# G1OJS/PyFT8

Hardware: AMD Instinct MI355X
Metric: FT8 15-s frames decoded/sec (higher is better)
Workload: dtype f32

## Files before the change

### pyft8_amd/csrc/kernels/common.hpp

```cpp
#ifndef FT8RX_COMMON_HPP
#define FT8RX_COMMON_HPP

struct Tables {
    const float* win;
    const cpx* W1920;
    const cpx* WR3840;
    const cpx* W3200;
    const cpx* W96000;
    const cpx* W300;
    const cpx* W320;
    const cpx* WR192k;
    const cpx* W32;
    const double* taper;
    const float* K32;
    const cpx* CS100;
    const cpx* TW100;
    const cpx* G1000;
};

__device__ __constant__ int d_COSTAS[7] = {3, 1, 4, 0, 6, 5, 2};
__device__ __constant__ uint8_t d_PAYSYM[58] = {7,8,9,10,11,12,13,14,15,16,17,18,19,20,21,22,23,24,25,26,27,28,29,30,31,32,33,34,35,
    43,44,45,46,47,48,49,50,51,52,53,54,55,56,57,58,59,60,61,62,63,64,65,66,67,68,69,70,71};
struct WorkList { int32_t* items; int32_t* count; };

constexpr __host__ __device__ int cand_shift(int max_cands) { return max_cands <= 256 ? 8 : max_cands <= 512 ? 9 : max_cands <= 1024 ? 10 : 11; }
constexpr __host__ __device__ int cand_shift(const ft8rx_config& c) { return cand_shift(c.max_cands); }
FT8_DEV bool cand_live(int c, int B, int sh, const int32_t* ncand) { return c < (B << sh) && (c & ((1 << sh) - 1)) < ncand[c >> sh]; }

FT8_DEV bool xcd_frame_map(int L, int per, int B, int& frame, int& idx) {
    const int x = L & 7, j = L >> 3;
    frame = 8 * (j / per) + x; idx = j % per;
    return frame < B;
}
#define XCD_GRID(B, per) ((((B) + 7) / 8) * 8 * (per))
enum { WL_BP0 = 0, WL_FINE = 1, WL_BP1 = 2, WL_BP1B = 3, WL_BP1C = 4, WL_OSD = 5, WL_OSDNAN = 6, WL_N = 7 };

#define W6 ((double)(-0.16666667163372040f))

#ifndef FT8RX_ILP_UNIT
__device__ __constant__ int8_t d_AP_CQ[29]   = {0,0,0,0,0, 0,0,0,0,0, 0,0,0,0,0, 0,0,0,0,0, 0,0,0,0,0, 0,1,0,0};
__device__ __constant__ int8_t d_AP_END[3][19] = {{0,1, 1,1,1,1,1, 0,0,1,1,1, 0,1,0,1,0, 0,1},
                                                  {0,1, 1,1,1,1,1, 0,1,0,0,1, 0,1,0,0,0, 0,1},
                                                  {0,1, 1,1,1,1,1, 0,1,0,0,1, 0,0,1,0,0, 0,1}};
__device__ uint8_t  d_CHK_N[83];
__device__ int16_t  d_CHK_V[83][7];
__device__ uint8_t  d_EDGE_V[522];
__device__ uint8_t  d_EDGE_C[522];
__device__ uint16_t d_VAR_E[174][3];
__device__ uint64_t d_G0[91][3];
__device__ uint64_t d_CHK_MASK[128][3];

struct Att {
    uint64_t lo, hi;
    int16_t n_its;
    uint8_t ok;
    uint8_t method;
    uint8_t nc0;
    uint8_t has_out;
    uint8_t pad[2];
};

FT8_DEV void work_push(const WorkList& w, int cand) { if (w.items) w.items[atomicAdd(w.count, 1)] = cand; }
FT8_DEV void work_push_block(const WorkList& w, bool want, int cand) {
    __shared__ int s_wave[4], s_base;
    const int lane = threadIdx.x & 63, wv = threadIdx.x >> 6;
    const uint64_t m = __ballot(want);
    if (lane == 0) s_wave[wv] = __popcll(m);
    __syncthreads();
    if (threadIdx.x == 0) {
        const int tot = s_wave[0] + s_wave[1] + s_wave[2] + s_wave[3];
        s_base = tot ? atomicAdd(w.count, tot) : 0;
    }
    __syncthreads();
    if (want) {
        int off = s_base + __popcll(m & ((1ull << lane) - 1));
        for (int i = 0; i < wv; i++) off += s_wave[i];
        w.items[off] = cand;
    }
}
FT8_DEV float grid_at(const float* __restrict__ g, int row, int col) {
    row %= 750; if (row < 0) row += 750;
    const bool in = row >= 1 && row <= 375;
    const uint32_t raw = __float_as_uint(g[(in ? row : 1) * FT8RX_GRID_COLS + col]);
    const uint32_t m = in ? 0xFFFFFFFFu : 0u;
    return __uint_as_float((raw & m) | (0x3F800000u & ~m));
}

FT8_DEV void log_event(ft8rx_event* ev, int32_t* evcount, int frame, int cand, int ipass, int slot, int seq,
                       uint64_t lo, uint64_t hi, int valid) {
    if (!ev) return;
    int idx = atomicAdd(&evcount[frame], 1);
    if (idx < FT8RX_EVENT_CAP) {
        ft8rx_event e; e.msg_lo = lo; e.msg_hi = hi; e.cand = (uint16_t)cand; e.ipass = (uint8_t)ipass;
        e.slot = (uint8_t)slot; e.seq = (uint16_t)seq; e.valid = (uint16_t)valid;
        ev[(size_t)frame * FT8RX_EVENT_CAP + idx] = e;
    }
}

__global__ __launch_bounds__(1024) void k_ev_scan(const int32_t* __restrict__ evcount, int B, int32_t* __restrict__ offs) {
    __shared__ int s_wave[16];
    __shared__ int s_carry;
    const int tid = threadIdx.x, lane = tid & 63, wv = tid >> 6;
    if (tid == 0) s_carry = 0;
    __syncthreads();
    for (int base = 0; base < B; base += 1024) {
        const int f = base + tid;
        int c = f < B ? evcount[f] : 0;
        c = c > FT8RX_EVENT_CAP ? FT8RX_EVENT_CAP : (c < 0 ? 0 : c);
        int incl = c;
#pragma unroll
        for (int d = 1; d < 64; d <<= 1) { const int t = __shfl_up(incl, d); if (lane >= d) incl += t; }
        if (lane == 63) s_wave[wv] = incl;
        __syncthreads();
        int before = s_carry;
        for (int i = 0; i < wv; i++) before += s_wave[i];
        if (f < B) offs[f] = before + incl - c;
        __syncthreads();
        if (tid == 1023) s_carry = before + incl;
        __syncthreads();
    }
    if (tid == 0) offs[B] = s_carry;
}
__global__ __launch_bounds__(64) void k_ev_compact(const ft8rx_event* __restrict__ ev, const int32_t* __restrict__ evcount,
                                                   const int32_t* __restrict__ offs, ft8rx_event* __restrict__ out) {
    const int f = blockIdx.x;
    int c = evcount[f]; c = c > FT8RX_EVENT_CAP ? FT8RX_EVENT_CAP : c;
    const uint32_t* src = reinterpret_cast<const uint32_t*>(ev + (size_t)f * FT8RX_EVENT_CAP);
    uint32_t* dst = reinterpret_cast<uint32_t*>(out + offs[f]);
    for (int i = threadIdx.x; i < c * 6; i += 64) dst[i] = src[i];
}

static_assert(sizeof(ft8rx_record) == 48 && sizeof(ft8rx_event) == 24 && sizeof(ft8rx_packed_frame) == 16 &&
              sizeof(ft8rx_packed_header) == 32, "packed result layout");
__global__ __launch_bounds__(256) void k_pack_count(const ft8rx_record* __restrict__ rec, const int32_t* __restrict__ ncand,
                                                    const ft8rx_event* __restrict__ ev, const int32_t* __restrict__ evcount,
                                                    uint64_t* __restrict__ need , int32_t* __restrict__ nrec , int sh) {
    __shared__ uint32_t s_has[FT8RX_MAX_CANDS / 32];
    __shared__ int s_cnt[FT8RX_MAX_CANDS / 64], s_nan;
    const int f = blockIdx.x, tid = threadIdx.x, lane = tid & 63, S = 1 << sh, nw = S >> 6;
    for (int i = tid; i < S / 32; i += 256) s_has[i] = 0;
    if (tid == 0) s_nan = 0;
    __syncthreads();
    int c = evcount[f]; c = c > FT8RX_EVENT_CAP ? FT8RX_EVENT_CAP : (c < 0 ? 0 : c);
    for (int i = tid; i < c; i += 256) {
        const unsigned cand = ev[(size_t)f * FT8RX_EVENT_CAP + i].cand;
        if (cand < (unsigned)S) atomicOr(&s_has[cand >> 5], 1u << (cand & 31));
    }
    int n = ncand[f]; n = n > S ? S : (n < 0 ? 0 : n);
    for (int i = tid; i < n; i += 256) {
        const ft8rx_record& r = rec[((size_t)f << sh) + i];
        if (r.grid_sd != r.grid_sd || r.fine_sd != r.fine_sd) s_nan = 1;
    }
    __syncthreads();
#pragma unroll 1
    for (int q = 0; q < S / 256; q++) {
        const int i = tid + 256 * q;
        const bool decoded = i < n && rec[((size_t)f << sh) + (i < n ? i : 0)].status == FT8RX_ST_DECODED;
        const bool want = i < n && (decoded || ((s_has[i >> 5] >> (i & 31)) & 1u) || s_nan);
        const uint64_t m = __ballot(want);
        if (lane == 0) { need[(size_t)f * nw + (i >> 6)] = m; s_cnt[i >> 6] = __popcll(m); }
    }
    __syncthreads();
    if (tid == 0) { int t = 0; for (int w = 0; w < nw; w++) t += s_cnt[w]; nrec[f] = t; }
}
__global__ __launch_bounds__(1024) void k_pack_scan(const int32_t* __restrict__ nrec, const int32_t* __restrict__ ncand,
                                                    const int32_t* __restrict__ evcount, int B, int max_cands, unsigned long long cap_bytes,
                                                    unsigned char* __restrict__ buf, ft8rx_packed_header* __restrict__ hdr_host) {
    __shared__ int s_wr[16], s_we[16];
    __shared__ int s_cr, s_ce;
    const int tid = threadIdx.x, lane = tid & 63, wv = tid >> 6;
    ft8rx_packed_frame* table = reinterpret_cast<ft8rx_packed_frame*>(buf + sizeof(ft8rx_packed_header));
    const bool table_fits = sizeof(ft8rx_packed_header) + (size_t)B * sizeof(ft8rx_packed_frame) <= cap_bytes;
    if (tid == 0) { s_cr = 0; s_ce = 0; }
    __syncthreads();
    for (int base = 0; base < B; base += 1024) {
        const int f = base + tid;
        const int r = f < B ? nrec[f] : 0;
        const int eraw = f < B ? evcount[f] : 0;
        const int e = eraw > FT8RX_EVENT_CAP ? FT8RX_EVENT_CAP : (eraw < 0 ? 0 : eraw);
        int ir = r, ie = e;
#pragma unroll
        for (int d = 1; d < 64; d <<= 1) { const int tr = __shfl_up(ir, d), te = __shfl_up(ie, d); if (lane >= d) { ir += tr; ie += te; } }
        if (lane == 63) { s_wr[wv] = ir; s_we[wv] = ie; }
        __syncthreads();
        int br = s_cr, be = s_ce;
        for (int i = 0; i < wv; i++) { br += s_wr[i]; be += s_we[i]; }
        if (f < B && table_fits) {
            ft8rx_packed_frame t;
            t.rec_off = br + ir - r; t.ev_off = be + ie - e;
            int n = ncand[f]; n = n > max_cands ? max_cands : (n < 0 ? 0 : n);
            t.n_cand = (uint16_t)n; t.n_rec = (uint16_t)r; t.n_ev = eraw < 0 ? 0 : eraw;
            table[f] = t;
        }
        __syncthreads();
        if (tid == 1023) { s_cr = br + ir; s_ce = be + ie; }
        __syncthreads();
    }
    if (tid == 0) {
        ft8rx_packed_header hd;
        hd.magic = FT8RX_PACKED_MAGIC; hd.n_frames = B; hd.n_records = s_cr; hd.n_events = s_ce; hd.max_cands = max_cands;
        hd.bytes = sizeof(ft8rx_packed_header) + (unsigned long long)B * sizeof(ft8rx_packed_frame) +
                   (unsigned long long)s_cr * sizeof(ft8rx_record) + (unsigned long long)s_ce * sizeof(ft8rx_event);
        hd.overflow = hd.bytes > cap_bytes;
        if (cap_bytes >= sizeof(hd)) *reinterpret_cast<ft8rx_packed_header*>(buf) = hd;
        *hdr_host = hd;
    }
}
__global__ __launch_bounds__(256) void k_pack_write(const ft8rx_record* __restrict__ rec, const ft8rx_event* __restrict__ ev,
                                                    const uint64_t* __restrict__ need, int B, unsigned char* __restrict__ buf, int sh) {
    const ft8rx_packed_header hd = *reinterpret_cast<const ft8rx_packed_header*>(buf);
    if (hd.overflow) return;
    __shared__ int s_pre[FT8RX_MAX_CANDS / 64];
    const int f = blockIdx.x, tid = threadIdx.x, lane = tid & 63, S = 1 << sh, nw = S >> 6;
    const ft8rx_packed_frame t = reinterpret_cast<const ft8rx_packed_frame*>(buf + sizeof(ft8rx_packed_header))[f];
    unsigned char* recs = buf + sizeof(ft8rx_packed_header) + (size_t)B * sizeof(ft8rx_packed_frame);
    unsigned char* evs = recs + (size_t)hd.n_records * sizeof(ft8rx_record);
    if (tid == 0) { int a = 0; for (int w = 0; w < nw; w++) { s_pre[w] = a; a += __popcll(need[(size_t)f * nw + w]); } }
    __syncthreads();
#pragma unroll 1
    for (int q = 0; q < S / 256; q++) {
        const int i = tid + 256 * q;
        const uint64_t mine = need[(size_t)f * nw + (i >> 6)];
        if ((mine >> lane) & 1ull) {
            const int p = s_pre[i >> 6] + __popcll(mine & ((1ull << lane) - 1));
            const uint4* src = reinterpret_cast<const uint4*>(rec + ((size_t)f << sh) + i);
            uint4* dst = reinterpret_cast<uint4*>(recs + ((size_t)t.rec_off + p) * sizeof(ft8rx_record));
            uint4 a = src[0], b = src[1], c = src[2];
            c.w = (uint32_t)i;
            dst[0] = a; dst[1] = b; dst[2] = c;
        }
    }
    const int ne = t.n_ev > FT8RX_EVENT_CAP ? FT8RX_EVENT_CAP : t.n_ev;
    const uint2* es = reinterpret_cast<const uint2*>(ev + (size_t)f * FT8RX_EVENT_CAP);
    uint2* ed = reinterpret_cast<uint2*>(evs + (size_t)t.ev_off * sizeof(ft8rx_event));
    for (int i = tid; i < ne * 3; i += 256) ed[i] = es[i];
}
#endif

#endif
```

### pyft8_amd/csrc/kernels/osd.hpp

```cpp
#ifndef FT8RX_OSD_HPP
#define FT8RX_OSD_HPP

#ifdef OSD_TIMING
__device__ unsigned long long g_osd_t[32768][10];
struct OsdClock { unsigned long long prev = __builtin_readcyclecounter(); };
#define OT(i) do { const unsigned long long ot_now = __builtin_readcyclecounter(); if (lane == 0) g_osd_t[blockIdx.x & 32767][i] += ot_now - ot.prev; ot.prev = __builtin_readcyclecounter(); } while (0)
#define OT_FLUSH do { if (lane == 0) g_osd_t[blockIdx.x & 32767][9] += 1ull; } while (0)
#else
struct OsdClock {};
#define OT(i) do { } while (0)
#define OT_FLUSH do { } while (0)
#endif
template <int M> FT8_DEV uint32_t osd_px(uint32_t v, int lane) {
    if (M == 1) return (uint32_t)__builtin_amdgcn_update_dpp(0, (int)v, 0xB1, 0xf, 0xf, false);
    if (M == 2) return (uint32_t)__builtin_amdgcn_update_dpp(0, (int)v, 0x4E, 0xf, 0xf, false);
    if (M == 3) return (uint32_t)__builtin_amdgcn_update_dpp(0, (int)v, 0x1B, 0xf, 0xf, false);
    if (M == 7) return (uint32_t)__builtin_amdgcn_update_dpp(0, (int)v, 0x141, 0xf, 0xf, false);
    if (M == 15) return (uint32_t)__builtin_amdgcn_update_dpp(0, (int)v, 0x140, 0xf, 0xf, false);
    if (M == 8) return (uint32_t)__builtin_amdgcn_update_dpp(0, (int)v, 0x128, 0xf, 0xf, false);
    if (M == 4 || M == 16 || M == 31) return (uint32_t)__builtin_amdgcn_ds_swizzle((int)v, 0x1f | (M << 10));
    return __shfl(v, lane ^ M);
}
#define OSD_LOWMASK(top) ((top) == 1 ? 0x5555555555555555ull : (top) == 2 ? 0x3333333333333333ull : (top) == 4 ? 0x0F0F0F0F0F0F0F0Full : \
                          (top) == 8 ? 0x00FF00FF00FF00FFull : (top) == 16 ? 0x0000FFFF0000FFFFull : 0x00000000FFFFFFFFull)
#define OSD_DPP_STAGE(CTRL)                                                                                                          \
    asm volatile("v_min_u32_dpp %[mn], %[hk], %[hk] " CTRL " row_mask:0xf bank_mask:0xf\n\t"                                         \
                 "v_max_u32_dpp %[mx], %[hk], %[hk] " CTRL " row_mask:0xf bank_mask:0xf\n\t"                                         \
                 "v_cndmask_b32 %[mn], %[mx], %[mn], %[low]\n\t"                                                                    \
                 "v_cmp_eq_u32 vcc, %[mn], %[hk]\n\t"                                                                                \
                 "s_nop 1\n\t"                                                                                                       \
                 "v_cndmask_b32_dpp %[ix], %[ix], %[ix], vcc " CTRL " row_mask:0xf bank_mask:0xf\n\t"                                \
                 : [mn] "=&v"(mn), [mx] "=&v"(mx), [ix] "+v"(ix[q]) : [hk] "v"(hk[q]), [low] "s"(low) : "vcc");
template <int M, int NQ> FT8_DEV void osd_stage(uint32_t* hk, uint32_t* ix, int lane) {
    constexpr int top = M >= 32 ? 32 : M >= 16 ? 16 : M >= 8 ? 8 : M >= 4 ? 4 : M >= 2 ? 2 : 1;
    const uint64_t low = OSD_LOWMASK(top);
#pragma unroll
    for (int q = 0; q < NQ; q++) {
        uint32_t mn, mx;
        if constexpr (M == 1) { OSD_DPP_STAGE("quad_perm:[1,0,3,2]") }
        else if constexpr (M == 2) { OSD_DPP_STAGE("quad_perm:[2,3,0,1]") }
        else if constexpr (M == 3) { OSD_DPP_STAGE("quad_perm:[3,2,1,0]") }
        else if constexpr (M == 7) { OSD_DPP_STAGE("row_half_mirror") }
        else if constexpr (M == 15) { OSD_DPP_STAGE("row_mirror") }
        else if constexpr (M == 8) { OSD_DPP_STAGE("row_ror:8") }
        else {
            const uint32_t pk = osd_px<M>(hk[q], lane), pi = osd_px<M>(ix[q], lane);
            mn = pk < hk[q] ? pk : hk[q]; mx = pk < hk[q] ? hk[q] : pk;
            asm("v_cndmask_b32 %0, %1, %0, %2" : "+v"(mn) : "v"(mx), "s"(low));
            ix[q] = (mn == hk[q]) ? ix[q] : pi;
        }
        hk[q] = mn;
    }
}
#undef OSD_DPP_STAGE
template <int NQ> FT8_DEV void osd_stages_421(uint32_t* hk, uint32_t* ix, int lane) {
    osd_stage<4, NQ>(hk, ix, lane); osd_stage<2, NQ>(hk, ix, lane); osd_stage<1, NQ>(hk, ix, lane);
}
template <bool REV> FT8_DEV void osd_stage_regs(uint32_t& ka, uint32_t& ia, uint32_t& kb, uint32_t& ib, int lane) {
    const uint32_t pkb = REV ? __shfl(kb, 63 - lane) : kb, pib = REV ? __shfl(ib, 63 - lane) : ib;
    const uint32_t pka = REV ? __shfl(ka, 63 - lane) : ka, pia = REV ? __shfl(ia, 63 - lane) : ia;
    const uint32_t na = pkb < ka ? pkb : ka, nb = pka > kb ? pka : kb;
    ia = (na == ka) ? ia : pib; ib = (nb == kb) ? ib : pia;
    ka = na; kb = nb;
}
#define FT8_HD __host__ __device__ inline
FT8_HD bool osd_nl(const float* x, int a, int b) {
    const float xa = x[a], xb = x[b];
    if (xa == xa && xb == xb) return fabsf(xa) > fabsf(xb);
    return xa == xa;
}
FT8_HD void osd_ss_linear_insert(const float* x, int* a, int last) {
    const int val = a[last]; int next = last - 1;
    while (osd_nl(x, val, a[next])) { a[last] = a[next]; last = next; next--; }
    a[last] = val;
}
FT8_HD void osd_ss_insertion(const float* x, int* a, int first, int last) {
    for (int i = first + 1; i < last; i++) {
        if (osd_nl(x, a[i], a[first])) { const int val = a[i]; for (int j = i; j > first; j--) a[j] = a[j - 1]; a[first] = val; }
        else osd_ss_linear_insert(x, a, i);
    }
}
FT8_HD void osd_ss_adjust_heap(const float* x, int* a, int first, int hole, int len, int value) {
    const int top = hole; int child = hole;
    while (child < (len - 1) / 2) {
        child = 2 * (child + 1);
        if (osd_nl(x, a[first + child], a[first + child - 1])) child--;
        a[first + hole] = a[first + child]; hole = child;
    }
    if ((len & 1) == 0 && child == (len - 2) / 2) { child = 2 * (child + 1); a[first + hole] = a[first + child - 1]; hole = child - 1; }
    int parent = (hole - 1) / 2;
    while (hole > top && osd_nl(x, a[first + parent], value)) { a[first + hole] = a[first + parent]; hole = parent; parent = (hole - 1) / 2; }
    a[first + hole] = value;
}
FT8_HD void osd_std_sort_withnan(const float* x, int* a, int* stack ) {
    const int n = 174;
    for (int i = 0; i < n; i++) a[i] = i;
    int sp = 0;
    stack[0] = 0; stack[1] = n; stack[2] = 2 * 7; sp = 1;
    while (sp > 0) {
        sp--;
        int first = stack[3 * sp], last = stack[3 * sp + 1], depth = stack[3 * sp + 2];
        while (last - first > 16) {
            if (depth == 0) {
                const int len = last - first;
                for (int parent = (len - 2) / 2; parent >= 0; parent--) osd_ss_adjust_heap(x, a, first, parent, len, a[first + parent]);
                while (last - first > 1) { last--; const int v = a[last]; a[last] = a[first]; osd_ss_adjust_heap(x, a, first, 0, last - first, v); }
                break;
            }
            depth--;
            {
                const int p = first + 1, q = first + (last - first) / 2, r = last - 1;
                int pick;
                if (osd_nl(x, a[p], a[q])) pick = osd_nl(x, a[q], a[r]) ? q : (osd_nl(x, a[p], a[r]) ? r : p);
                else pick = osd_nl(x, a[p], a[r]) ? p : (osd_nl(x, a[q], a[r]) ? r : q);
                const int t = a[first]; a[first] = a[pick]; a[pick] = t;
            }
            int lo = first + 1, hi = last;
            for (;;) {
                while (osd_nl(x, a[lo], a[first])) lo++;
                hi--;
                while (osd_nl(x, a[first], a[hi])) hi--;
                if (!(lo < hi)) break;
                const int t = a[lo]; a[lo] = a[hi]; a[hi] = t;
                lo++;
            }
            stack[3 * sp] = lo; stack[3 * sp + 1] = last; stack[3 * sp + 2] = depth; sp++;
            last = lo;
        }
    }
    osd_ss_insertion(x, a, 0, 16);
    for (int i = 16; i < n; i++) osd_ss_linear_insert(x, a, i);
}

#undef FT8_HD
__device__ uint8_t d_NANPERM[192];

#define OSD_MAXFLIP 91
#define OSD_FLIPS_A 62
#define OSD_MAXTRIALS 16384
#define OSD_NONE 0xFFu

__device__ __constant__ uint32_t d_SYNM[14][3];
__device__ uint32_t d_G0T[192][3];

struct OsdArgs {
    const float* llr_in; const float* saved; const Att* attB; ft8rx_record* rec; const int32_t* ncand; Att* attO;
    ft8rx_event* ev; int32_t* evcount; const uint32_t* trials; int ntr, nflip, max_hd, sh; WorkList nanlist; unsigned mt; const ApCalls* apc;
};

struct OsdLds {
    float llr[176];
    uint64_t work[256];
    uint64_t ftab[192];
    uint32_t hmw[3];
    uint16_t fsyn[OSD_MAXFLIP + 2];
    FT8_DEV int* ordl() { return reinterpret_cast<int*>(work); }
    FT8_DEV int* posrow() { return reinterpret_cast<int*>(work); }
    FT8_DEV uint32_t* ftabB() { return reinterpret_cast<uint32_t*>(work); }
    FT8_DEV int* frow() { return reinterpret_cast<int*>(work) + 192; }
};
static_assert(176 + 3 * 20 <= 512 && 192 + OSD_MAXFLIP <= 512 && sizeof(OsdLds) <= 4496, "the overlays fit the 512 words of work[]; 4.5 KB per block");

struct OsdInput { bool go; int slot; size_t vec; const float* hsrc; };
template <bool AP7>
FT8_DEV OsdInput osd_load(OsdLds& L, int lane, int mode, int bid, const OsdArgs& a) {
    OsdInput in = {true, 0, (size_t)bid, L.llr};
    if constexpr (AP7) {
        in.slot = bid & 15; const size_t c = (size_t)(bid >> 4);
        in.hsrc = a.llr_in + c * 174;
        const float v0 = in.hsrc[lane], v1 = in.hsrc[64 + lane], v2 = in.hsrc[128 + (lane < 46 ? lane : 0)];
        L.llr[lane] = ap7_value(a.apc, in.slot, lane, v0); L.llr[64 + lane] = ap7_value(a.apc, in.slot, 64 + lane, v1);
        if (lane < 46) L.llr[128 + lane] = ap7_value(a.apc, in.slot, 128 + lane, v2);
        in.vec = c * 10 + (in.slot - 5);
    } else if (mode == 0) {
        const int slot = in.slot = bid % 10; const int c = bid / 10;
        in.go = false;
        if ((c & ((1 << a.sh) - 1)) >= a.ncand[c >> a.sh]) return in;
        if (a.rec[c].status != FT8RX_ST_ACTIVE) return in;
        if (slot >= 5 && !a.attB[(size_t)c * 5 + (slot - 5)].has_out) { if (lane == 0) { Att u; memset(&u, 0, sizeof(u)); u.n_its = -1; a.attO[(size_t)c * 10 + slot] = u; } return in; }
        in.go = true;
        const float* src = slot < 5 ? a.llr_in + (size_t)c * 174 : a.saved + ((size_t)c * 5 + (slot - 5)) * 174;
        const int apx = slot < 5 ? slot : 0;
        const float v0 = src[lane], v1 = src[64 + lane], v2 = src[128 + (lane < 46 ? lane : 0)];
        L.llr[lane] = ap_value(apx, lane, v0); L.llr[64 + lane] = ap_value(apx, 64 + lane, v1);
        if (lane < 46) L.llr[128 + lane] = ap_value(apx, 128 + lane, v2);
        in.vec = (size_t)c * 10 + slot;
    } else {
        for (int i = lane; i < 174; i += 64) L.llr[i] = a.llr_in[in.vec * 174 + i];
    }
    __syncthreads();
    return in;
}

template <bool NANV>
FT8_DEV bool osd_order(OsdLds& L, int lane, int bid, const WorkList& nanlist, uint32_t* ix, OsdClock& ot) {
    uint32_t hk[3];
#pragma unroll
    for (int q = 0; q < 3; q++) {
        const int i = lane + 64 * q;
        const uint32_t mag = __float_as_uint(L.llr[i < 174 ? i : 0]) & 0x7fffffffu;
        hk[q] = (i < 174) ? 0xFFFFFFFEu - mag : 0xFFFFFFFFu;
        ix[q] = (i < 174) ? (uint32_t)i : 0u;
    }
    const uint64_t nan0 = __ballot(hk[0] < 0x807FFFFEu), nan1 = __ballot(hk[1] < 0x807FFFFEu), nan2 = __ballot(lane < 46 && hk[2] < 0x807FFFFEu);
    const bool any_nan = (nan0 | nan1 | nan2) != 0, all_nan = (nan0 & nan1) == ~0ull && nan2 == (1ull << 46) - 1;
    OT(0);
    if (NANV) {
        if (!any_nan || all_nan) return false;
        int* ordl = L.ordl();
        if (lane == 0) osd_std_sort_withnan(L.llr, ordl, ordl + 176);
        __syncthreads();
        ix[0] = (uint32_t)ordl[lane]; ix[1] = (uint32_t)ordl[64 + lane]; ix[2] = (uint32_t)ordl[128 + (lane < 46 ? lane : 0)];
        __syncthreads();
    } else if (all_nan) {
        ix[0] = d_NANPERM[lane]; ix[1] = d_NANPERM[64 + lane]; ix[2] = d_NANPERM[128 + lane];
    } else if (any_nan) {
        if (lane == 0) work_push(nanlist, bid);
        return false;
    } else {
        osd_stage<1, 3>(hk, ix, lane); osd_stage<3, 3>(hk, ix, lane); osd_stage<1, 3>(hk, ix, lane);
        osd_stage<7, 3>(hk, ix, lane); osd_stage<2, 3>(hk, ix, lane); osd_stage<1, 3>(hk, ix, lane);
        osd_stage<15, 3>(hk, ix, lane); osd_stages_421<3>(hk, ix, lane);
        osd_stage<31, 3>(hk, ix, lane); osd_stage<8, 3>(hk, ix, lane); osd_stages_421<3>(hk, ix, lane);
        osd_stage<63, 3>(hk, ix, lane); osd_stage<16, 3>(hk, ix, lane); osd_stage<8, 3>(hk, ix, lane); osd_stages_421<3>(hk, ix, lane);
        osd_stage_regs<true>(hk[0], ix[0], hk[1], ix[1], lane);
        osd_stage<32, 2>(hk, ix, lane); osd_stage<16, 2>(hk, ix, lane); osd_stage<8, 2>(hk, ix, lane); osd_stages_421<2>(hk, ix, lane);
        osd_stage_regs<true>(hk[1], ix[1], hk[2], ix[2], lane);
        osd_stage_regs<false>(hk[0], ix[0], hk[1], ix[1], lane);
        osd_stage<32, 3>(hk, ix, lane); osd_stage<16, 3>(hk, ix, lane); osd_stage<8, 3>(hk, ix, lane); osd_stages_421<3>(hk, ix, lane);
    }
    return true;
}

struct OsdHard { uint64_t w0, w1, w2; };
FT8_DEV OsdHard osd_hard(const float* v, int lane) {
    return {__ballot(v[lane] > 0.0f), __ballot(v[64 + lane] > 0.0f), __ballot(lane < 46 && v[128 + (lane < 46 ? lane : 0)] > 0.0f)};
}

struct OsdBasis {
    uint32_t x00, x01, x02, x10, x11, x12, x20, x21, x22;
    uint64_t acc0, acc1, acc2;
    bool hs0, hs1, hs2;
};
FT8_DEV OsdBasis osd_eliminate(OsdLds& L, int lane, const uint32_t* ix, OsdClock& ot) {
    const int ord0 = (int)ix[0], ord1 = (int)ix[1], ord2 = (lane < 46) ? (int)ix[2] : 0;
    const bool has2 = lane < 46;
    uint32_t x00 = d_G0T[ord0][0], x01 = d_G0T[ord0][1], x02 = d_G0T[ord0][2];
    uint32_t x10 = d_G0T[ord1][0], x11 = d_G0T[ord1][1], x12 = d_G0T[ord1][2];
    uint32_t x20 = has2 ? d_G0T[ord2][0] : 0u, x21 = has2 ? d_G0T[ord2][1] : 0u, x22 = has2 ? d_G0T[ord2][2] : 0u;
    const bool hs0 = L.llr[ord0] > 0.0f, hs1 = L.llr[ord1] > 0.0f, hs2 = has2 && L.llr[ord2] > 0.0f;
    uint64_t acc0 = 0, acc1 = 0, acc2 = 0;
    int k = 0;
#define OSD_TRIV 96
    int* posrow = L.posrow();
    if (ord0 < 91) posrow[ord0] = lane;
    if (ord1 < 91) posrow[ord1] = 64 + lane;
    if (has2 && ord2 < 91) posrow[ord2] = 128 + lane;
    uint64_t triv0 = __ballot(ord0 < 91), triv1 = __ballot(ord1 < 91 && lane < OSD_TRIV - 64);
    int tc0 = __builtin_amdgcn_mbcnt_hi((uint32_t)(triv0 >> 32), __builtin_amdgcn_mbcnt_lo((uint32_t)triv0, 0));
    int tc1 = __popcll(triv0) + __builtin_amdgcn_mbcnt_hi((uint32_t)(triv1 >> 32), __builtin_amdgcn_mbcnt_lo((uint32_t)triv1, 0));
    int ntriv = __popcll(triv0) + __popcll(triv1);
    __syncthreads();
    const uint64_t u01 = __ballot(posrow[lane] < OSD_TRIV);
    const uint32_t u2 = (uint32_t)__ballot(lane < 27 && posrow[64 + (lane < 27 ? lane : 0)] < OSD_TRIV);
    uint64_t vis0 = ~triv0, vis1 = ~triv1, vis2 = (1ull << 46) - 1;
#define OSD_UPD(XW, X0, X1, X2) { const uint32_t mk = (uint32_t)__builtin_amdgcn_sbfe((int)(XW), bp, 1u); X0 ^= mk & m0; X1 ^= mk & m1; X2 ^= mk & m2; }
#define OSD_STEP(XA, XB, XC, ACC, VIS, TCV, BASE, UPD0, UPD1, UPD2)                                                                \
    while (VIS != 0) {                                                                                                             \
        const int il = __builtin_ctzll(VIS);                                                                                       \
        if (k + __builtin_amdgcn_readlane(TCV, il) >= 91) { vis0 = 0; vis1 = 0; vis2 = 0; continue; }       \
        const uint64_t bit = 1ull << il;                                                                                           \
        VIS &= ~bit; ACC |= bit; k++;                                                                                              \
        const uint32_t c0 = __builtin_amdgcn_readlane(XA, il), c1 = __builtin_amdgcn_readlane(XB, il), c2 = __builtin_amdgcn_readlane(XC, il); \
        uint32_t a0 = c0 & ~lockU0, a1 = c1 & ~lockU1, a2 = c2 & ~lockU2;                                                          \
        if (__builtin_expect(!(a0 | a1 | a2), 0)) {             \
            const int p = (BASE) + il;                                                                                             \
             \
            const int pa = posrow[lane], pb = posrow[64 + (lane < 27 ? lane : 0)];                                                 \
            const bool ta = pa > p && pa < OSD_TRIV && (((pa < 64 ? triv0 >> pa : triv1 >> (pa - 64)) & 1ull) != 0);               \
            const bool tb = lane < 27 && pb > p && pb < OSD_TRIV && (((pb < 64 ? triv0 >> pb : triv1 >> (pb - 64)) & 1ull) != 0);  \
            const uint64_t s01 = (((uint64_t)c1 << 32) | c0) & __ballot(ta);                                                       \
            a0 = (uint32_t)s01; a1 = (uint32_t)(s01 >> 32); a2 = c2 & (uint32_t)__ballot(tb);                                      \
            if (a0 | a1 | a2) {                                                                                                    \
                const int r = s01 ? __builtin_ctzll(s01) : 64 + __builtin_ctz(a2);                                                 \
                const int q = __builtin_amdgcn_readfirstlane(posrow[r]);    \
                if (q < 64) { triv0 &= ~(1ull << q); vis0 |= 1ull << q; tc0 -= (lane > q) ? 1 : 0; tc1 -= 1; }                    \
                else { triv1 &= ~(1ull << (q - 64)); vis1 |= 1ull << (q - 64); tc1 -= (lane > q - 64) ? 1 : 0; }                   \
                ntriv--;                                                                                                           \
            } else { ACC &= ~bit; k--; }                                                    \
        }                                                                                                                          \
        asm volatile("" : "+s"(a2));                            \
                        \
        if (a0) {                                                                                                                  \
            const uint32_t b = a0 & (0u - a0), bp = __builtin_ctz(a0), m0 = c0 & ~b, m1 = c1, m2 = c2;                             \
            UPD0                                                                                                                   \
            lockU0 |= b;                                                                                                           \
        } else if (a1) {                                                                                                           \
            const uint32_t b = a1 & (0u - a1), bp = __builtin_ctz(a1), m0 = c0, m1 = c1 & ~b, m2 = c2;                             \
            UPD1                                                                                                                   \
            lockU1 |= b;                                                                                                           \
        } else {                                                \
            const uint32_t b = a2 & (0u - a2), bp = __builtin_ctz(a2 | 0x80000000u), m0 = c0, m1 = c1, m2 = c2 & ~b;               \
            UPD2                                                                                                                   \
            lockU2 |= b;                                                                                                           \
        }                                                                                                                          \
    }
    uint32_t lockU0 = (uint32_t)u01, lockU1 = (uint32_t)(u01 >> 32), lockU2 = ~((1u << 27) - 1u) | u2;
    OT(2);
    OSD_STEP(x00, x01, x02, acc0, vis0, tc0, 0,
             OSD_UPD(x00, x00, x01, x02) OSD_UPD(x10, x10, x11, x12) OSD_UPD(x20, x20, x21, x22),
             OSD_UPD(x01, x00, x01, x02) OSD_UPD(x11, x10, x11, x12) OSD_UPD(x21, x20, x21, x22),
             OSD_UPD(x02, x00, x01, x02) OSD_UPD(x12, x10, x11, x12) OSD_UPD(x22, x20, x21, x22))
    OSD_STEP(x10, x11, x12, acc1, vis1, tc1, 64,
             OSD_UPD(x10, x10, x11, x12) OSD_UPD(x20, x20, x21, x22),
             OSD_UPD(x11, x10, x11, x12) OSD_UPD(x21, x20, x21, x22),
             OSD_UPD(x12, x10, x11, x12) OSD_UPD(x22, x20, x21, x22))
    {
        int tc2 = ntriv;
        OSD_STEP(x20, x21, x22, acc2, vis2, tc2, 128, OSD_UPD(x20, x20, x21, x22), OSD_UPD(x21, x20, x21, x22), OSD_UPD(x22, x20, x21, x22))
    }
#undef OSD_STEP
#undef OSD_UPD
    acc0 |= __ballot(((triv0 >> lane) & 1ull) && tc0 < 91 - k);
    acc1 |= __ballot(((triv1 >> lane) & 1ull) && tc1 < 91 - k);
    __syncthreads();
    return {x00, x01, x02, x10, x11, x12, x20, x21, x22, acc0, acc1, acc2, hs0, hs1, hs2};
}

template <bool WIDE>
FT8_DEV void osd_flip_table(OsdLds& L, int lane, const uint32_t* ix, const OsdBasis& b, int nflip, OsdClock& ot) {
    const int nflipA = WIDE ? OSD_FLIPS_A : nflip;
    const bool has2 = lane < 46;
    const int ord0 = (int)ix[0], ord1 = (int)ix[1], ord2 = has2 ? (int)ix[2] : 0;
    const bool in0 = (b.acc0 >> lane) & 1ull, in1 = (b.acc1 >> lane) & 1ull, in2 = (b.acc2 >> lane) & 1ull;
    const int n0 = __popcll(b.acc0), n1 = __popcll(b.acc1);
    const int kk0 = __builtin_amdgcn_mbcnt_hi((uint32_t)(b.acc0 >> 32), __builtin_amdgcn_mbcnt_lo((uint32_t)b.acc0, 0));
    const int kk1 = n0 + __builtin_amdgcn_mbcnt_hi((uint32_t)(b.acc1 >> 32), __builtin_amdgcn_mbcnt_lo((uint32_t)b.acc1, 0));
    const int kk2 = n0 + n1 + __builtin_amdgcn_mbcnt_hi((uint32_t)(b.acc2 >> 32), __builtin_amdgcn_mbcnt_lo((uint32_t)b.acc2, 0));
    int* fri = L.frow();
#define OSD_ROWIDX(X0, X1, X2) ((X0) ? __builtin_ctz(X0) : (X1) ? 32 + __builtin_ctz(X1) : 64 + __builtin_ctz((X2) | 0x80000000u))
    { const int i = 90 - kk0; if (in0 && i >= 0 && i < nflip) fri[i] = OSD_ROWIDX(b.x00, b.x01, b.x02); }
    { const int i = 90 - kk1; if (in1 && i >= 0 && i < nflip) fri[i] = OSD_ROWIDX(b.x10, b.x11, b.x12); }
    { const int i = 90 - kk2; if (in2 && i >= 0 && i < nflip) fri[i] = OSD_ROWIDX(b.x20, b.x21, b.x22); }
#undef OSD_ROWIDX
    if (lane < 3) L.hmw[lane] = 0u;
    __syncthreads();
    {
        const uint32_t h0 = ((in0 && b.hs0) ? b.x00 : 0u) | ((in1 && b.hs1) ? b.x10 : 0u) | ((in2 && b.hs2) ? b.x20 : 0u);
        const uint32_t h1 = ((in0 && b.hs0) ? b.x01 : 0u) | ((in1 && b.hs1) ? b.x11 : 0u) | ((in2 && b.hs2) ? b.x21 : 0u);
        const uint32_t h2 = ((in0 && b.hs0) ? b.x02 : 0u) | ((in1 && b.hs1) ? b.x12 : 0u) | ((in2 && b.hs2) ? b.x22 : 0u);
        if (h0) atomicOr(&L.hmw[0], h0);
        if (h1) atomicOr(&L.hmw[1], h1);
        if (h2) atomicOr(&L.hmw[2], h2);
    }
    __syncthreads();
    const uint32_t hm0 = L.hmw[0], hm1 = L.hmw[1], hm2 = L.hmw[2];
    OT(4);
    uint32_t f0l = 0, f1l = 0, f2l = 0;
    uint32_t f0h = (uint32_t)((__popc(b.x00 & hm0) + __popc(b.x01 & hm1) + __popc(b.x02 & hm2)) & 1) << 31,
             f1h = (uint32_t)((__popc(b.x10 & hm0) + __popc(b.x11 & hm1) + __popc(b.x12 & hm2)) & 1) << 31,
             f2h = (uint32_t)((__popc(b.x20 & hm0) + __popc(b.x21 & hm1) + __popc(b.x22 & hm2)) & 1) << 31;
#define OSD_FBIT(XA, XB, XC, FA, FB, FC, SH) { FA |= __builtin_amdgcn_ubfe(XA, bp, 1u) << (SH); FB |= __builtin_amdgcn_ubfe(XB, bp, 1u) << (SH); \
                                               FC |= __builtin_amdgcn_ubfe(XC, bp, 1u) << (SH); }
#define OSD_FLIPS(LO, HI, FA, FB, FC, SUB)                                                                                         \
    for (int i = (LO); i < (HI); i++) {                                                                                            \
        const int r = __builtin_amdgcn_readfirstlane(fri[i]);                                                                      \
        const uint32_t bp = (uint32_t)r & 31u, sh = (uint32_t)(i - (SUB));                                                         \
        if (r < 32) OSD_FBIT(b.x00, b.x10, b.x20, FA, FB, FC, sh)                                                                  \
        else if (r < 64) OSD_FBIT(b.x01, b.x11, b.x21, FA, FB, FC, sh)                                                             \
        else OSD_FBIT(b.x02, b.x12, b.x22, FA, FB, FC, sh)                                                                         \
    }
    OSD_FLIPS(0, nflipA < 32 ? nflipA : 32, f0l, f1l, f2l, 0)
    OSD_FLIPS(32, nflipA, f0h, f1h, f2h, 32)
    L.ftab[ord0] = ((uint64_t)f0h << 32) | f0l; L.ftab[ord1] = ((uint64_t)f1h << 32) | f1l; if (has2) L.ftab[ord2] = ((uint64_t)f2h << 32) | f2l;
    if (WIDE) {
        uint32_t* ftabB = L.ftabB();
        uint32_t g0 = 0, g1 = 0, g2 = 0;
        OSD_FLIPS(OSD_FLIPS_A, nflip, g0, g1, g2, OSD_FLIPS_A)
        ftabB[ord0] = g0; ftabB[ord1] = g1; if (has2) ftabB[ord2] = g2;
    }
#undef OSD_FLIPS
#undef OSD_FBIT
    __syncthreads();
}

template <class Bit> FT8_DEV unsigned osd_syndrome_of(Bit bit) {
    uint32_t ra = 0, rb = 0, rc = 0;
#pragma unroll 8
    for (int v = 0; v < 32; v++) { ra |= bit(v) << v; rb |= bit(32 + v) << v; rc |= bit(64 + (v < 27 ? v : 0)) << v; }
    rc &= (1u << 27) - 1;
    unsigned sy = 0;
#pragma unroll
    for (int k = 0; k < 14; k++)
        sy |= (unsigned)((__popc(ra & d_SYNM[k][0]) + __popc(rb & d_SYNM[k][1]) + __popc(rc & d_SYNM[k][2])) & 1) << k;
    return sy;
}
template <bool WIDE>
FT8_DEV void osd_syndromes(OsdLds& L, int lane, int nflip) {
    const int nflipA = WIDE ? OSD_FLIPS_A : nflip;
    const int bitsel = (lane < nflipA) ? lane : 63;
    const uint32_t* fh = reinterpret_cast<const uint32_t*>(L.ftab) + (bitsel >= 32 ? 1 : 0);
    const unsigned sy = osd_syndrome_of([&](int v) { return __builtin_amdgcn_ubfe(fh[2 * v], (uint32_t)bitsel & 31u, 1u); });
    if (lane < nflipA) L.fsyn[lane] = (uint16_t)sy;
    if (lane == 63) L.fsyn[OSD_MAXFLIP + 1] = (uint16_t)sy;
    if (lane == 0) L.fsyn[OSD_MAXFLIP] = 0;
    if (WIDE) {
        const uint32_t* ftabB = L.ftabB();
        const unsigned syB = osd_syndrome_of([&](int v) { return (ftabB[v] >> (lane & 31)) & 1u; });
        if (OSD_FLIPS_A + lane < nflip) L.fsyn[OSD_FLIPS_A + lane] = (uint16_t)syB;
    }
    __syncthreads();
}

template <bool WIDE, bool EXT, bool AP7>
FT8_DEV Att osd_trials(OsdLds& L, int lane, const OsdInput& in, const OsdHard& hard, const OsdArgs& a) {
    const bool has2 = lane < 46;
    const uint32_t* ftabB = L.ftabB();
    const unsigned syn_c = L.fsyn[OSD_MAXFLIP + 1];
    const uint64_t M1 = (1ull << 27) - 1, M2 = (1ull << 46) - 1;
    Att res; memset(&res, 0, sizeof(res)); res.n_its = -1;
    const int slot = in.slot, ipass = AP7 ? 7 : (slot < 5) ? 5 : 6;
    for (int base = 0; base < a.ntr; base += 64) {
        const int t = base + lane;
        bool hit = false; int i = OSD_MAXFLIP, j = OSD_MAXFLIP, q = OSD_MAXFLIP;
        if (t < a.ntr) {
            const uint32_t e = a.trials[t];
            i = e & 0xFF; j = (e >> 8) & 0xFF; q = (e >> 16) & 0xFF;
            if (i == OSD_NONE) i = OSD_MAXFLIP;
            if (j == OSD_NONE) j = OSD_MAXFLIP;
            if (q == OSD_NONE) q = OSD_MAXFLIP;
            hit = (syn_c ^ L.fsyn[i] ^ L.fsyn[j] ^ L.fsyn[q]) == 0;
        }
        uint64_t hits = __ballot(hit);
        if (!hits) continue;
        bool done = false;
        while (hits && !done) {
            const int hl = __builtin_ctzll(hits);
            hits &= hits - 1;
            const int hi_ = __shfl(i, hl), hj = __shfl(j, hl), hq = __shfl(q, hl);
            const uint64_t msk = (1ull << 63) | ((hi_ < OSD_FLIPS_A) ? (1ull << hi_) : 0ull) | ((hj < OSD_FLIPS_A) ? (1ull << hj) : 0ull) |
                                 ((hq < OSD_FLIPS_A) ? (1ull << hq) : 0ull);
            uint32_t mskB = 0;
            if (WIDE) mskB = ((hi_ >= OSD_FLIPS_A && hi_ < OSD_MAXFLIP) ? (1u << (hi_ - OSD_FLIPS_A)) : 0u) |
                             ((hj >= OSD_FLIPS_A && hj < OSD_MAXFLIP) ? (1u << (hj - OSD_FLIPS_A)) : 0u) |
                             ((hq >= OSD_FLIPS_A && hq < OSD_MAXFLIP) ? (1u << (hq - OSD_FLIPS_A)) : 0u);
            const int l2 = 128 + (has2 ? lane : 0);
            const int pb0 = WIDE ? __popc(ftabB[lane] & mskB) : 0, pb1 = WIDE ? __popc(ftabB[64 + lane] & mskB) : 0, pb2 = WIDE ? __popc(ftabB[l2] & mskB) : 0;
            const uint64_t w0 = __ballot((__popcll(L.ftab[lane] & msk) + pb0) & 1), w1 = __ballot((__popcll(L.ftab[64 + lane] & msk) + pb1) & 1),
                           w2 = __ballot(has2 && ((__popcll(L.ftab[l2] & msk) + pb2) & 1));
            const int hd = __popcll(w0 ^ hard.w0) + __popcll(w1 ^ hard.w1) + __popcll((w2 ^ hard.w2) & M2);
            if (a.max_hd > 0 && hd > a.max_hd) continue;
            uint64_t lo = 0, hi = 0;
            const int r = ft8_crc_check<EXT>(w0, w1 & M1, &lo, &hi, a.mt, true);
            const int t = base + hl;
            if (r && lane == 0) log_event(a.ev, a.evcount, (int)(in.vec / 10) >> a.sh, (int)(in.vec / 10) & ((1 << a.sh) - 1), ipass, AP7 ? 2 * slot + 1 : slot, t, lo, hi, r == 2);
            if (r == 2) {
                res.ok = 1; res.lo = lo; res.hi = hi; res.n_its = (int16_t)t;
                if constexpr (AP7) res.ok = hd <= a.apc->max_hd;
                res.method = (AP7 || slot < 5) ? FT8RX_M_OSD : FT8RX_M_LDPC_B_OSD;
                res.pad[0] = (uint8_t)hd;
                done = true;
            }
        }
        if (done) break;
    }
    return res;
}

template <bool WIDE, bool NANV, bool EXT = false, bool AP7 = false>
FT8_DEV void osd_attempt(int lane, int mode, int bid, const OsdArgs& a) {
    __shared__ OsdLds L;
    OsdClock ot;
    const OsdInput in = osd_load<AP7>(L, lane, mode, bid, a);
    if (!in.go) return;
    uint32_t ix[3];
    if (!osd_order<NANV>(L, lane, bid, a.nanlist, ix, ot)) return;
    OT(1);
    const OsdHard hard = osd_hard(in.hsrc, lane);
    const OsdBasis basis = osd_eliminate(L, lane, ix, ot);
    OT(3);
    osd_flip_table<WIDE>(L, lane, ix, basis, a.nflip, ot);
    OT(5);
    osd_syndromes<WIDE>(L, lane, a.nflip);
    OT(6);
    const Att res = osd_trials<WIDE, EXT, AP7>(L, lane, in, hard, a);
    OT(7);
    if (lane == 0) a.attO[in.vec] = res;
    OT_FLUSH;
}

#ifndef OSD_ATTR
#define OSD_ATTR __attribute__((amdgpu_waves_per_eu(8, 8)))
#endif
template <bool WIDE, bool NANV, bool EXT, bool AP7, class Id>
FT8_DEV void osd_blocks(int n, int mode, const OsdArgs& a, Id id) {
#pragma unroll 1
    for (int item = blockIdx.x; item < n; item += gridDim.x) {
        int lane = threadIdx.x;
        asm volatile("" : "+v"(lane));
        osd_attempt<WIDE, NANV, EXT, AP7>(lane, mode, id(item), a);
        __syncthreads();
    }
}
#define OSD_PARAMS int mode, const float* __restrict__ llr_in, const float* __restrict__ saved, const Att* __restrict__ attB,       \
                   ft8rx_record* __restrict__ rec, const int32_t* __restrict__ ncand, Att* __restrict__ attO, ft8rx_event* ev,      \
                   int32_t* evcount, const uint32_t* __restrict__ trials, int ntr, int nflip, int max_hd, int sh
#define OSD_KERNEL(NAME, NAN_NAME, WIDE, EXT, MT_PARAM, MT)                                                                          \
__global__ __launch_bounds__(64) OSD_ATTR void NAME(OSD_PARAMS, WorkList work, WorkList nanlist MT_PARAM) {                         \
    const OsdArgs a = {llr_in, saved, attB, rec, ncand, attO, ev, evcount, trials, ntr, nflip, max_hd, sh, nanlist, MT, nullptr};   \
    osd_blocks<WIDE, false, EXT, false>(mode == 2 ? (int)gridDim.x : *work.count * 10, mode, a,                                     \
                                        [&](int item) { return mode == 2 ? item : work.items[item / 10] * 10 + item % 10; });       \
}                                                                                                                                   \
__global__ __launch_bounds__(64) void NAN_NAME(OSD_PARAMS, WorkList nanlist MT_PARAM) {                                             \
    const OsdArgs a = {llr_in, saved, attB, rec, ncand, attO, ev, evcount, trials, ntr, nflip, max_hd, sh, nanlist, MT, nullptr};   \
    osd_blocks<WIDE, true, EXT, false>(*nanlist.count, mode, a, [&](int item) { return nanlist.items[item]; });                     \
}
#define OSD_MT_PARAM , unsigned mt
OSD_KERNEL(k_osd, k_osd_nan, false, false, , 0u)
OSD_KERNEL(k_osd_wide, k_osd_nan_wide, true, false, , 0u)
OSD_KERNEL(k_osd_ext, k_osd_nan_ext, false, true, OSD_MT_PARAM, mt)
OSD_KERNEL(k_osd_wide_ext, k_osd_nan_wide_ext, true, true, OSD_MT_PARAM, mt)
#undef OSD_KERNEL
#undef OSD_PARAMS
#undef OSD_MT_PARAM
#define OSD_NAN_GRID 512

#endif
```

Measured before the change: 88430.

## Share OSD elimination across AP end-variant slots 2-4 in one block

Slots 2, 3 and 4 differ only in the AP end pattern on bits 58-76. They now share one ordering, elimination and flip table, and the block runs the trials for all three variants in sequence. Each extra variant gets its own hard-decision mask, folded into the flip table as extra columns (bits 62 and 61 of the high word), so OSD_FLIPS_A drops from 62 to 61. The grid shrinks from 10 to 8 items per candidate, and LDS per block grows somewhat. The risk is that the shared reliability ordering differs from what each variant would have computed on its own AP-modified LLRs, and that the bits freed for variants reduce flip capacity.

```diff
diff --git a/pyft8_amd/csrc/kernels/common.hpp b/pyft8_amd/csrc/kernels/common.hpp
--- a/pyft8_amd/csrc/kernels/common.hpp
+++ b/pyft8_amd/csrc/kernels/common.hpp
@@ -39,9 +39,10 @@
 
 #ifndef FT8RX_ILP_UNIT
 __device__ __constant__ int8_t d_AP_CQ[29]   = {0,0,0,0,0, 0,0,0,0,0, 0,0,0,0,0, 0,0,0,0,0, 0,0,0,0,0, 0,1,0,0};
-__device__ __constant__ int8_t d_AP_END[3][19] = {{0,1, 1,1,1,1,1, 0,0,1,1,1, 0,1,0,1,0, 0,1},
-                                                  {0,1, 1,1,1,1,1, 0,1,0,0,1, 0,1,0,0,0, 0,1},
-                                                  {0,1, 1,1,1,1,1, 0,1,0,0,1, 0,0,1,0,0, 0,1}};
+#define FT8_AP_END_ROWS {0,1, 1,1,1,1,1, 0,0,1,1,1, 0,1,0,1,0, 0,1}, \
+                        {0,1, 1,1,1,1,1, 0,1,0,0,1, 0,1,0,0,0, 0,1}, \
+                        {0,1, 1,1,1,1,1, 0,1,0,0,1, 0,0,1,0,0, 0,1}
+__device__ __constant__ int8_t d_AP_END[3][19] = {FT8_AP_END_ROWS};
 __device__ uint8_t  d_CHK_N[83];
 __device__ int16_t  d_CHK_V[83][7];
 __device__ uint8_t  d_EDGE_V[522];
diff --git a/pyft8_amd/csrc/kernels/osd.hpp b/pyft8_amd/csrc/kernels/osd.hpp
--- a/pyft8_amd/csrc/kernels/osd.hpp
+++ b/pyft8_amd/csrc/kernels/osd.hpp
@@ -6,10 +6,12 @@
 struct OsdClock { unsigned long long prev = __builtin_readcyclecounter(); };
 #define OT(i) do { const unsigned long long ot_now = __builtin_readcyclecounter(); if (lane == 0) g_osd_t[blockIdx.x & 32767][i] += ot_now - ot.prev; ot.prev = __builtin_readcyclecounter(); } while (0)
 #define OT_FLUSH do { if (lane == 0) g_osd_t[blockIdx.x & 32767][9] += 1ull; } while (0)
+#define OT_ATTEMPT do { if (lane == 0) g_osd_t[blockIdx.x & 32767][8] += 1ull; } while (0)
 #else
 struct OsdClock {};
 #define OT(i) do { } while (0)
 #define OT_FLUSH do { } while (0)
+#define OT_ATTEMPT do { } while (0)
 #endif
 template <int M> FT8_DEV uint32_t osd_px(uint32_t v, int lane) {
     if (M == 1) return (uint32_t)__builtin_amdgcn_update_dpp(0, (int)v, 0xB1, 0xf, 0xf, false);
@@ -136,7 +138,8 @@
 __device__ uint8_t d_NANPERM[192];
 
 #define OSD_MAXFLIP 91
-#define OSD_FLIPS_A 62
+#define OSD_FLIPS_A 61
+#define OSD_NVAR 3
 #define OSD_MAXTRIALS 16384
 #define OSD_NONE 0xFFu
 
@@ -152,19 +155,29 @@
     float llr[176];
     uint64_t work[256];
     uint64_t ftab[192];
-    uint32_t hmw[3];
-    uint16_t fsyn[OSD_MAXFLIP + 2];
+    uint32_t hmw[OSD_NVAR][3];
+    uint16_t fsyn[OSD_MAXFLIP + 1 + OSD_NVAR];
     FT8_DEV int* ordl() { return reinterpret_cast<int*>(work); }
     FT8_DEV int* posrow() { return reinterpret_cast<int*>(work); }
     FT8_DEV uint32_t* ftabB() { return reinterpret_cast<uint32_t*>(work); }
     FT8_DEV int* frow() { return reinterpret_cast<int*>(work) + 192; }
 };
-static_assert(176 + 3 * 20 <= 512 && 192 + OSD_MAXFLIP <= 512 && sizeof(OsdLds) <= 4496, "the overlays fit the 512 words of work[]; 4.5 KB per block");
-
-struct OsdInput { bool go; int slot; size_t vec; const float* hsrc; };
-template <bool AP7>
+static_assert(176 + 3 * 20 <= 512 && 192 + OSD_MAXFLIP <= 512 && sizeof(OsdLds) <= 5120, "the overlays fit the 512 words of work[]; 32 blocks (8 waves per SIMD) in 160 KB");
+
+struct OsdInput { bool go; int slot; size_t vec; const float* hsrc; int nvar; };
+constexpr uint32_t osd_ap_end_row(int v) {
+    constexpr int8_t rows[3][19] = {FT8_AP_END_ROWS};
+    uint32_t w = 0;
+    for (int i = 0; i < 19; i++) w |= (uint32_t)(rows[v][i] != 0) << i;
+    return w;
+}
+FT8_DEV uint32_t osd_ap_end_word(int v) {
+    constexpr uint32_t w1 = osd_ap_end_row(1), w2 = osd_ap_end_row(2);
+    return v == 1 ? w1 : w2;
+}
+template <bool AP7, bool SHARE>
 FT8_DEV OsdInput osd_load(OsdLds& L, int lane, int mode, int bid, const OsdArgs& a) {
-    OsdInput in = {true, 0, (size_t)bid, L.llr};
+    OsdInput in = {true, 0, (size_t)bid, L.llr, 1};
     if constexpr (AP7) {
         in.slot = bid & 15; const size_t c = (size_t)(bid >> 4);
         in.hsrc = a.llr_in + c * 174;
@@ -185,6 +198,7 @@
         L.llr[lane] = ap_value(apx, lane, v0); L.llr[64 + lane] = ap_value(apx, 64 + lane, v1);
         if (lane < 46) L.llr[128 + lane] = ap_value(apx, 128 + lane, v2);
         in.vec = (size_t)c * 10 + slot;
+        if (SHARE && slot == 2) in.nvar = OSD_NVAR;
     } else {
         for (int i = lane; i < 174; i += 64) L.llr[i] = a.llr_in[in.vec * 174 + i];
     }
@@ -193,7 +207,7 @@
 }
 
 template <bool NANV>
-FT8_DEV bool osd_order(OsdLds& L, int lane, int bid, const WorkList& nanlist, uint32_t* ix, OsdClock& ot) {
+FT8_DEV bool osd_order(OsdLds& L, int lane, int bid, int nvar, const WorkList& nanlist, uint32_t* ix, OsdClock& ot) {
     uint32_t hk[3];
 #pragma unroll
     for (int q = 0; q < 3; q++) {
@@ -215,7 +229,7 @@
     } else if (all_nan) {
         ix[0] = d_NANPERM[lane]; ix[1] = d_NANPERM[64 + lane]; ix[2] = d_NANPERM[128 + lane];
     } else if (any_nan) {
-        if (lane == 0) work_push(nanlist, bid);
+        if (lane == 0) for (int v = 0; v < nvar; v++) work_push(nanlist, bid + v);
         return false;
     } else {
         osd_stage<1, 3>(hk, ix, lane); osd_stage<3, 3>(hk, ix, lane); osd_stage<1, 3>(hk, ix, lane);
@@ -328,7 +342,7 @@
 }
 
 template <bool WIDE>
-FT8_DEV void osd_flip_table(OsdLds& L, int lane, const uint32_t* ix, const OsdBasis& b, int nflip, OsdClock& ot) {
+FT8_DEV void osd_flip_table(OsdLds& L, int lane, const uint32_t* ix, const OsdBasis& b, int nflip, int nvar, OsdClock& ot) {
     const int nflipA = WIDE ? OSD_FLIPS_A : nflip;
     const bool has2 = lane < 46;
     const int ord0 = (int)ix[0], ord1 = (int)ix[1], ord2 = has2 ? (int)ix[2] : 0;
@@ -343,18 +357,18 @@
     { const int i = 90 - kk1; if (in1 && i >= 0 && i < nflip) fri[i] = OSD_ROWIDX(b.x10, b.x11, b.x12); }
     { const int i = 90 - kk2; if (in2 && i >= 0 && i < nflip) fri[i] = OSD_ROWIDX(b.x20, b.x21, b.x22); }
 #undef OSD_ROWIDX
-    if (lane < 3) L.hmw[lane] = 0u;
+    if (lane < 3 * OSD_NVAR) (&L.hmw[0][0])[lane] = 0u;
     __syncthreads();
     {
         const uint32_t h0 = ((in0 && b.hs0) ? b.x00 : 0u) | ((in1 && b.hs1) ? b.x10 : 0u) | ((in2 && b.hs2) ? b.x20 : 0u);
         const uint32_t h1 = ((in0 && b.hs0) ? b.x01 : 0u) | ((in1 && b.hs1) ? b.x11 : 0u) | ((in2 && b.hs2) ? b.x21 : 0u);
         const uint32_t h2 = ((in0 && b.hs0) ? b.x02 : 0u) | ((in1 && b.hs1) ? b.x12 : 0u) | ((in2 && b.hs2) ? b.x22 : 0u);
-        if (h0) atomicOr(&L.hmw[0], h0);
-        if (h1) atomicOr(&L.hmw[1], h1);
-        if (h2) atomicOr(&L.hmw[2], h2);
-    }
-    __syncthreads();
-    const uint32_t hm0 = L.hmw[0], hm1 = L.hmw[1], hm2 = L.hmw[2];
+        if (h0) atomicOr(&L.hmw[0][0], h0);
+        if (h1) atomicOr(&L.hmw[0][1], h1);
+        if (h2) atomicOr(&L.hmw[0][2], h2);
+    }
+    __syncthreads();
+    const uint32_t hm0 = L.hmw[0][0], hm1 = L.hmw[0][1], hm2 = L.hmw[0][2];
     OT(4);
     uint32_t f0l = 0, f1l = 0, f2l = 0;
     uint32_t f0h = (uint32_t)((__popc(b.x00 & hm0) + __popc(b.x01 & hm1) + __popc(b.x02 & hm2)) & 1) << 31,
@@ -372,6 +386,27 @@
     }
     OSD_FLIPS(0, nflipA < 32 ? nflipA : 32, f0l, f1l, f2l, 0)
     OSD_FLIPS(32, nflipA, f0h, f1h, f2h, 32)
+    if (nvar > 1) {
+#pragma unroll 1
+        for (int v = 1; v < nvar; v++) {
+            const uint32_t p = osd_ap_end_word(v), d0 = (uint32_t)(ord0 - 58), d1 = (uint32_t)(ord1 - 58), d2 = (uint32_t)(ord2 - 58);
+            const bool s0 = d0 < 19u ? (p >> d0) & 1u : b.hs0, s1 = d1 < 19u ? (p >> d1) & 1u : b.hs1, s2 = d2 < 19u ? (p >> d2) & 1u : b.hs2;
+            const uint32_t h0 = ((in0 && s0) ? b.x00 : 0u) | ((in1 && s1) ? b.x10 : 0u) | ((in2 && s2) ? b.x20 : 0u);
+            const uint32_t h1 = ((in0 && s0) ? b.x01 : 0u) | ((in1 && s1) ? b.x11 : 0u) | ((in2 && s2) ? b.x21 : 0u);
+            const uint32_t h2 = ((in0 && s0) ? b.x02 : 0u) | ((in1 && s1) ? b.x12 : 0u) | ((in2 && s2) ? b.x22 : 0u);
+            if (h0) atomicOr(&L.hmw[v][0], h0);
+            if (h1) atomicOr(&L.hmw[v][1], h1);
+            if (h2) atomicOr(&L.hmw[v][2], h2);
+        }
+        __syncthreads();
+#pragma unroll 1
+        for (int v = 1; v < nvar; v++) {
+            const uint32_t gm0 = L.hmw[v][0], gm1 = L.hmw[v][1], gm2 = L.hmw[v][2];
+            f0h |= (uint32_t)((__popc(b.x00 & gm0) + __popc(b.x01 & gm1) + __popc(b.x02 & gm2)) & 1) << (31 - v);
+            f1h |= (uint32_t)((__popc(b.x10 & gm0) + __popc(b.x11 & gm1) + __popc(b.x12 & gm2)) & 1) << (31 - v);
+            f2h |= (uint32_t)((__popc(b.x20 & gm0) + __popc(b.x21 & gm1) + __popc(b.x22 & gm2)) & 1) << (31 - v);
+        }
+    }
     L.ftab[ord0] = ((uint64_t)f0h << 32) | f0l; L.ftab[ord1] = ((uint64_t)f1h << 32) | f1l; if (has2) L.ftab[ord2] = ((uint64_t)f2h << 32) | f2l;
     if (WIDE) {
         uint32_t* ftabB = L.ftabB();
@@ -398,11 +433,11 @@
 template <bool WIDE>
 FT8_DEV void osd_syndromes(OsdLds& L, int lane, int nflip) {
     const int nflipA = WIDE ? OSD_FLIPS_A : nflip;
-    const int bitsel = (lane < nflipA) ? lane : 63;
+    const int bitsel = lane;
     const uint32_t* fh = reinterpret_cast<const uint32_t*>(L.ftab) + (bitsel >= 32 ? 1 : 0);
     const unsigned sy = osd_syndrome_of([&](int v) { return __builtin_amdgcn_ubfe(fh[2 * v], (uint32_t)bitsel & 31u, 1u); });
     if (lane < nflipA) L.fsyn[lane] = (uint16_t)sy;
-    if (lane == 63) L.fsyn[OSD_MAXFLIP + 1] = (uint16_t)sy;
+    if (lane > 63 - OSD_NVAR) L.fsyn[OSD_MAXFLIP + 1 + (63 - lane)] = (uint16_t)sy;
     if (lane == 0) L.fsyn[OSD_MAXFLIP] = 0;
     if (WIDE) {
         const uint32_t* ftabB = L.ftabB();
@@ -413,10 +448,10 @@
 }
 
 template <bool WIDE, bool EXT, bool AP7>
-FT8_DEV Att osd_trials(OsdLds& L, int lane, const OsdInput& in, const OsdHard& hard, const OsdArgs& a) {
+FT8_DEV Att osd_trials(OsdLds& L, int lane, const OsdInput& in, const OsdHard& hard, int var, const OsdArgs& a) {
     const bool has2 = lane < 46;
     const uint32_t* ftabB = L.ftabB();
-    const unsigned syn_c = L.fsyn[OSD_MAXFLIP + 1];
+    const unsigned syn_c = L.fsyn[OSD_MAXFLIP + 1 + var];
     const uint64_t M1 = (1ull << 27) - 1, M2 = (1ull << 46) - 1;
     Att res; memset(&res, 0, sizeof(res)); res.n_its = -1;
     const int slot = in.slot, ipass = AP7 ? 7 : (slot < 5) ? 5 : 6;
@@ -438,7 +473,7 @@
             const int hl = __builtin_ctzll(hits);
             hits &= hits - 1;
             const int hi_ = __shfl(i, hl), hj = __shfl(j, hl), hq = __shfl(q, hl);
-            const uint64_t msk = (1ull << 63) | ((hi_ < OSD_FLIPS_A) ? (1ull << hi_) : 0ull) | ((hj < OSD_FLIPS_A) ? (1ull << hj) : 0ull) |
+            const uint64_t msk = (1ull << (63 - var)) | ((hi_ < OSD_FLIPS_A) ? (1ull << hi_) : 0ull) | ((hj < OSD_FLIPS_A) ? (1ull << hj) : 0ull) |
                                  ((hq < OSD_FLIPS_A) ? (1ull << hq) : 0ull);
             uint32_t mskB = 0;
             if (WIDE) mskB = ((hi_ >= OSD_FLIPS_A && hi_ < OSD_MAXFLIP) ? (1u << (hi_ - OSD_FLIPS_A)) : 0u) |
@@ -471,21 +506,31 @@
 FT8_DEV void osd_attempt(int lane, int mode, int bid, const OsdArgs& a) {
     __shared__ OsdLds L;
     OsdClock ot;
-    const OsdInput in = osd_load<AP7>(L, lane, mode, bid, a);
+    OsdInput in = osd_load<AP7, !NANV && !AP7>(L, lane, mode, bid, a);
     if (!in.go) return;
     uint32_t ix[3];
-    if (!osd_order<NANV>(L, lane, bid, a.nanlist, ix, ot)) return;
+    if (!osd_order<NANV>(L, lane, bid, in.nvar, a.nanlist, ix, ot)) return;
     OT(1);
-    const OsdHard hard = osd_hard(in.hsrc, lane);
+    OsdHard hard = osd_hard(in.hsrc, lane);
     const OsdBasis basis = osd_eliminate(L, lane, ix, ot);
     OT(3);
-    osd_flip_table<WIDE>(L, lane, ix, basis, a.nflip, ot);
+    osd_flip_table<WIDE>(L, lane, ix, basis, a.nflip, in.nvar, ot);
     OT(5);
     osd_syndromes<WIDE>(L, lane, a.nflip);
     OT(6);
-    const Att res = osd_trials<WIDE, EXT, AP7>(L, lane, in, hard, a);
-    OT(7);
-    if (lane == 0) a.attO[in.vec] = res;
+#pragma unroll 1
+    for (int v = 0; v < in.nvar; v++) {
+        if (v) {
+            const uint32_t p = osd_ap_end_word(v);
+            hard.w0 = (hard.w0 & ~(0x3Full << 58)) | ((uint64_t)(p & 0x3Fu) << 58);
+            hard.w1 = (hard.w1 & ~0x1FFFull) | (uint64_t)(p >> 6);
+            in.slot++; in.vec++;
+        }
+        const Att res = osd_trials<WIDE, EXT, AP7>(L, lane, in, hard, v, a);
+        OT(7);
+        if (lane == 0) a.attO[in.vec] = res;
+        OT_ATTEMPT;
+    }
     OT_FLUSH;
 }
 
@@ -502,14 +547,16 @@
         __syncthreads();
     }
 }
+#define OSD_ITEMS 8
+#define OSD_ITEM_SLOT(i) ((i) < 3 ? (i) : (i) + 2)
 #define OSD_PARAMS int mode, const float* __restrict__ llr_in, const float* __restrict__ saved, const Att* __restrict__ attB,       \
                    ft8rx_record* __restrict__ rec, const int32_t* __restrict__ ncand, Att* __restrict__ attO, ft8rx_event* ev,      \
                    int32_t* evcount, const uint32_t* __restrict__ trials, int ntr, int nflip, int max_hd, int sh
 #define OSD_KERNEL(NAME, NAN_NAME, WIDE, EXT, MT_PARAM, MT)                                                                          \
 __global__ __launch_bounds__(64) OSD_ATTR void NAME(OSD_PARAMS, WorkList work, WorkList nanlist MT_PARAM) {                         \
     const OsdArgs a = {llr_in, saved, attB, rec, ncand, attO, ev, evcount, trials, ntr, nflip, max_hd, sh, nanlist, MT, nullptr};   \
-    osd_blocks<WIDE, false, EXT, false>(mode == 2 ? (int)gridDim.x : *work.count * 10, mode, a,                                     \
-                                        [&](int item) { return mode == 2 ? item : work.items[item / 10] * 10 + item % 10; });       \
+    osd_blocks<WIDE, false, EXT, false>(mode == 2 ? (int)gridDim.x : *work.count * OSD_ITEMS, mode, a,                              \
+                                        [&](int item) { return mode == 2 ? item : work.items[item / OSD_ITEMS] * 10 + OSD_ITEM_SLOT(item % OSD_ITEMS); }); \
 }                                                                                                                                   \
 __global__ __launch_bounds__(64) void NAN_NAME(OSD_PARAMS, WorkList nanlist MT_PARAM) {                                             \
     const OsdArgs a = {llr_in, saved, attB, rec, ncand, attO, ev, evcount, trials, ntr, nflip, max_hd, sh, nanlist, MT, nullptr};   \
```

Measured after the change: 89570, median of 6. 1.3% higher.
